# mmetcalf14/qml-cutensornet

Hardware: AMD Instinct MI355X
Metric: Gram kernel entries/sec @ 60 qubits x 6 layers (higher is better)
Workload: dtype f64 (complex128)

## Files before the change

### qml-cutensornet_amd/csrc/qk_fused.h

```cpp
#pragma once
#include "qk_device.h"

#define QKF_PRIO_LO() __builtin_amdgcn_s_setprio(0)
#define QKF_PRIO_HI() __builtin_amdgcn_s_setprio(2)
typedef double v2d __attribute__((ext_vector_type(2)));
typedef __attribute__((address_space(3))) v2d lds_v2d;
static constexpr int QKF_XSTEP = 4 * TILE;
static constexpr int QKF_XBLOCK = TILE * TILE;


#ifndef QKF_LDS3M
#define QKF_LDS3M 0
#endif
#ifndef QKF_P2_PROBE
#define QKF_P2_PROBE 0
#endif
#ifndef QKF_ABL
#define QKF_ABL 0
#endif
#define QKF_STEP_BARRIER()                            \
  do {                                                \
    if (QKF_ABL & 4) asm volatile("s_waitcnt lgkmcnt(0)" ::: "memory"); \
    else qk_lds_barrier();                            \
  } while (0)
#define QKF_SUM(a, b) ((QKF_ABL & 1) ? (a) : (a) + (b))
#define QKF_DIF(a, b) ((QKF_ABL & 1) ? (b) : (a) - (b))
template <bool CONJB>
__device__ __forceinline__ void qkf_kstep(v4d& p1, v4d& p2, v4d& p3, const double ar, const double ai, const double br, const double bi) {
  const double sa = QKF_SUM(ar, ai), sb = CONJB ? QKF_DIF(br, bi) : QKF_SUM(br, bi);
  p1 = __builtin_amdgcn_mfma_f64_16x16x4f64(ar, br, p1, 0, 0, 0);
  p2 = __builtin_amdgcn_mfma_f64_16x16x4f64(ai, bi, p2, 0, 0, 0);
  p3 = __builtin_amdgcn_mfma_f64_16x16x4f64(sa, sb, p3, 0, 0, 0);
}

struct QkfTile {
  v4d re, im;
};

__device__ __forceinline__ v2d qkf_ldg(const v2d* __restrict__ base, const unsigned off) {
  return *reinterpret_cast<const v2d*>(reinterpret_cast<const char*>(base) + (size_t)(off * 16u));
}
#ifndef QKF_NT_A
#define QKF_NT_A 0
#endif
#ifndef QKF_NT_B
#define QKF_NT_B 0
#endif
__device__ __forceinline__ v2d qkf_ldg_nt(const v2d* __restrict__ base, const unsigned off) {
  return __builtin_nontemporal_load(reinterpret_cast<const v2d*>(reinterpret_cast<const char*>(base) + (size_t)(off * 16u)));
}
__device__ __forceinline__ v2d qkf_ldg_a(const v2d* __restrict__ base, const unsigned off) { return QKF_NT_A ? qkf_ldg_nt(base, off) : qkf_ldg(base, off); }
__device__ __forceinline__ v2d qkf_ldg_b(const v2d* __restrict__ base, const unsigned off) { return QKF_NT_B ? qkf_ldg_nt(base, off) : qkf_ldg(base, off); }
__device__ __forceinline__ v2d qkf_ldx(const v2d* __restrict__ base, const unsigned off) { return qkf_ldg(base, off); }
__device__ __forceinline__ v2d qkf_ldx(const lds_v2d* base, const unsigned off) { return base[off]; }

struct QkfStream {
  const v2d* base;
  unsigned off;
  int step;
};
__device__ __forceinline__ void qkf_load4(v2d (&fr)[4], const QkfStream& st) {
#pragma unroll
  for (int i = 0; i < 4; ++i) fr[i] = qkf_ldg(st.base + i * st.step, st.off);
}

template <typename XPtr>
__device__ __forceinline__ void qkf_p1_tile(QkfTile& t, v2d (&fr)[4], const bool primed, QkfStream cur, XPtr xp, unsigned xoff, const int nks, const QkfStream nxt) {
  v4d p1 = {0, 0, 0, 0}, p2 = {0, 0, 0, 0}, p3 = {0, 0, 0, 0};
  v2d fx[4];
  if (!primed) qkf_load4(fr, cur);
#pragma unroll
  for (int i = 0; i < 4; ++i) fx[i] = qkf_ldx(xp + i * QKF_XSTEP, xoff);
  const int ng = (nks + 3) >> 2, last = nks - 4 * (ng - 1);
  QKF_PRIO_LO();
  int gq = 0;
  if (ng >= 2) {
    gq = 1;
    cur.off += 4 * cur.step, xoff += 4 * QKF_XSTEP;
#pragma unroll
    for (int i = 0; i < 4; ++i) {
      if (i == 0) {
        const v4d z = {0, 0, 0, 0};
        p1 = __builtin_amdgcn_mfma_f64_16x16x4f64(fx[0].x, fr[0].x, z, 0, 0, 0);
        p2 = __builtin_amdgcn_mfma_f64_16x16x4f64(fx[0].y, fr[0].y, z, 0, 0, 0);
        p3 = __builtin_amdgcn_mfma_f64_16x16x4f64(QKF_SUM(fx[0].x, fx[0].y), QKF_SUM(fr[0].x, fr[0].y), z, 0, 0, 0);
      } else {
        qkf_kstep<false>(p1, p2, p3, fx[i].x, fx[i].y, fr[i].x, fr[i].y);
      }
      if (!(QKF_ABL & 2)) fr[i] = qkf_ldg_b(cur.base + i * cur.step, cur.off);
      if (!(QKF_ABL & 8)) fx[i] = qkf_ldx(xp + i * QKF_XSTEP, xoff);
      __builtin_amdgcn_sched_barrier(0);
    }
  }
#pragma unroll 1
  for (; gq + 1 < ng; ++gq) {
    cur.off += 4 * cur.step, xoff += 4 * QKF_XSTEP;
#pragma unroll
    for (int i = 0; i < 4; ++i) {
      qkf_kstep<false>(p1, p2, p3, fx[i].x, fx[i].y, fr[i].x, fr[i].y);
      if (!(QKF_ABL & 2)) fr[i] = qkf_ldg_b(cur.base + i * cur.step, cur.off);
      if (!(QKF_ABL & 8)) fx[i] = qkf_ldx(xp + i * QKF_XSTEP, xoff);
      __builtin_amdgcn_sched_barrier(0);
    }
  }
#pragma unroll
  for (int i = 0; i < 4; ++i) {
    if (i < last) qkf_kstep<false>(p1, p2, p3, fx[i].x, fx[i].y, fr[i].x, fr[i].y);
    if (!(QKF_ABL & 2)) fr[i] = qkf_ldg(nxt.base + i * nxt.step, nxt.off);
    __builtin_amdgcn_sched_barrier(0);
  }
  QKF_PRIO_HI();
  t.re = p1 - p2;
  t.im = p3 - p1 - p2;
}

typedef __attribute__((address_space(3))) int lds_int;
struct QkfTurn {
  lds_int* at;
  int idx;
  lds_int* broken;
  unsigned long long* gerr;
};
__device__ __forceinline__ void qkf_turn_add(__attribute__((address_space(3))) double* const d, const long rs, const v4d& re, const v4d& im, const QkfTurn& t, const int tn) {
  lds_int* const turn = t.at + tn;
  if (t.idx > 0) {
    int spins = 0;
#ifdef QKF_FIRST_STORE
    while (__builtin_amdgcn_readfirstlane(__hip_atomic_load(turn, __ATOMIC_RELAXED, __HIP_MEMORY_SCOPE_WORKGROUP)) == 0) {
#else
    while (__builtin_amdgcn_readfirstlane(__hip_atomic_load(turn, __ATOMIC_RELAXED, __HIP_MEMORY_SCOPE_WORKGROUP)) != t.idx) {
#endif
      __builtin_amdgcn_s_sleep(1);
      if (++spins > (1 << 20) || __builtin_amdgcn_readfirstlane(__hip_atomic_load(t.broken, __ATOMIC_RELAXED, __HIP_MEMORY_SCOPE_WORKGROUP)) != 0) {
        __hip_atomic_store(t.broken, 1, __ATOMIC_RELAXED, __HIP_MEMORY_SCOPE_WORKGROUP);
        if (t.gerr) *t.gerr = 1ull;
        break;
      }
    }
#pragma unroll
    for (int r = 0; r < 4; ++r) {
      __hip_atomic_fetch_add(d + r * rs, re[r], __ATOMIC_RELAXED, __HIP_MEMORY_SCOPE_WORKGROUP);
      __hip_atomic_fetch_add(d + r * rs + 1, im[r], __ATOMIC_RELAXED, __HIP_MEMORY_SCOPE_WORKGROUP);
    }
  } else {
#pragma unroll
    for (int r = 0; r < 4; ++r) *(lds_v2d*)(d + r * rs) = (v2d){re[r], im[r]};
  }
#ifdef QKF_FIRST_STORE
  if (t.idx > 0) return;
#endif
  asm volatile("s_waitcnt lgkmcnt(0)" ::: "memory");
  __hip_atomic_store(turn, t.idx + 1, __ATOMIC_RELAXED, __HIP_MEMORY_SCOPE_WORKGROUP);
}

template <bool FULL, bool DET = false>
__device__ __forceinline__ void qkf_p2_item(const QkfTile& t, v2d (&fr)[4], const bool primed, QkfStream cur, const int ps, const int nn, const int kmax, lds_v2d* xo, const int q,
                                            const int j, const QkfStream nxt, const QkfTurn turn = QkfTurn{nullptr, 0, nullptr, nullptr}) {
  if (!primed) qkf_load4(fr, cur);
  __attribute__((address_space(3))) double* d = (__attribute__((address_space(3))) double*)(xo + q * TILE + j);
#pragma unroll 1
  for (int tn = 0; tn < nn; ++tn) {
    v4d p1 = {0, 0, 0, 0}, p2 = {0, 0, 0, 0}, p3 = {0, 0, 0, 0};
    const bool fin = tn + 1 == nn;
    const v2d* const rb = fin ? nxt.base : cur.base;
    const int rs = fin ? nxt.step : cur.step;
    cur.off = fin ? nxt.off : cur.off + TILE;
    QKF_PRIO_LO();
#pragma unroll
    for (int i = 0; i < 4; ++i) {
      if (FULL || i < kmax) qkf_kstep<true>(p1, p2, p3, t.re[i], t.im[i], fr[i].x, fr[i].y);
      if (!(QKF_ABL & 2)) fr[i] = qkf_ldg_a(rb + i * rs, cur.off);
      __builtin_amdgcn_sched_barrier(0);
    }
    QKF_PRIO_HI();
    const v4d re = (QKF_ABL & 128) ? p1 : p1 + p2, im = (QKF_ABL & 128) ? p3 : p3 - p1 + p2;
    if constexpr (DET) qkf_turn_add(d, (long)2 * QKF_XSTEP, re, im, turn, tn);
    else if (QKF_ABL & 256) {
#pragma unroll
      for (int r = 0; r < 4; ++r) asm volatile("" ::"v"(re[r]), "v"(im[r]));
    } else {
#pragma unroll
      for (int r = 0; r < 4; ++r) {
        __hip_atomic_fetch_add(d + r * 2 * QKF_XSTEP, re[r], __ATOMIC_RELAXED, __HIP_MEMORY_SCOPE_WORKGROUP);
        __hip_atomic_fetch_add(d + r * 2 * QKF_XSTEP + 1, im[r], __ATOMIC_RELAXED, __HIP_MEMORY_SCOPE_WORKGROUP);
      }
    }
    d += 2 * ps;
  }
}

template <int S>
__device__ __forceinline__ void qkf_rotate(QkfTile (&T)[S], const int L) {
  if constexpr (S >= 2) {
    if (L == 2) {
      const QkfTile t = T[S - 2];
      T[S - 2] = T[S - 1], T[S - 1] = t;
    }
  }
  if constexpr (S >= 3) {
    if (L == 3) {
      const QkfTile t = T[S - 3];
      T[S - 3] = T[S - 2], T[S - 2] = T[S - 1], T[S - 1] = t;
    }
  }
  if constexpr (S >= 4) {
    if (L >= 4) {
      const QkfTile t0 = T[0];
#pragma unroll
      for (int e = 0; e + 1 < S; ++e) T[e] = T[e + 1];
      T[S - 1] = t0;
    }
  }
}

__device__ __forceinline__ void qkf_edge_tile(QkfTile& t, const v2d* __restrict__ Ay, const int ldy, const v2d* __restrict__ Ax, const int ldx, const int ks4) {
  v4d p1 = {0, 0, 0, 0}, p2 = {0, 0, 0, 0}, p3 = {0, 0, 0, 0};
  v2d fy[4], fx[4];
#pragma unroll
  for (int i = 0; i < 4; ++i) fy[i] = Ay[(long)(4 * i) * ldy], fx[i] = Ax[(long)(4 * i) * ldx];
  for (int s0 = 0; s0 < ks4; s0 += 4) {
    const bool more = s0 + 4 < ks4;
#pragma unroll
    for (int i = 0; i < 4; ++i) {
      qkf_kstep<true>(p1, p2, p3, fy[i].x, fy[i].y, fx[i].x, fx[i].y);
      if (more) fy[i] = Ay[(long)(4 * (s0 + 4 + i)) * ldy], fx[i] = Ax[(long)(4 * (s0 + 4 + i)) * ldx];
    }
  }
  t.re = p1 + p2, t.im = p3 - p1 + p2;
}

template <int NW, typename XOut>
__device__ __forceinline__ void qkf_edge_prefix(const SweepArgs& g, const int xi, const int yj, const int a, const int b, XOut xo, const int wave, const int q, const int j) {
  const v2d* const Lx = reinterpret_cast<const v2d*>(g.xedge) + g.xedge_offs[2 * (long long)xi];
  const v2d* const Ly = reinterpret_cast<const v2d*>(g.yedge) + g.yedge_offs[2 * (long long)yj];
  const int mt = a / TILE, nt = b / TILE, ks4 = (1 << g.edge_k) >> 2;
  for (int t = wave; t < mt * nt; t += NW) {
    const int tb = t / mt, ta = t - tb * mt;
    QkfTile T;
    qkf_edge_tile(T, Ly + (long)q * b + tb * TILE + j, b, Lx + (long)q * a + ta * TILE + j, a, ks4);
#pragma unroll
    for (int r = 0; r < 4; ++r) xo[ta * (b * TILE) + (tb * TILE + q + 4 * r) * TILE + j] = (v2d){T.re[r], T.im[r]};
  }
}

template <int NW, typename XIn>
__device__ __forceinline__ void qkf_edge_suffix(const SweepArgs& g, const int xi, const int yj, const int a, const int b, XIn xin, __attribute__((address_space(3))) double* zacc, const int wave,
                                                const int q, const int j) {
  const v2d* const Rx = reinterpret_cast<const v2d*>(g.xedge) + g.xedge_offs[2 * (long long)xi + 1];
  const v2d* const Ry = reinterpret_cast<const v2d*>(g.yedge) + g.yedge_offs[2 * (long long)yj + 1];
  const int mt = a / TILE, nt = b / TILE, ks4 = (1 << g.edge_k) >> 2;
  double zr = 0, zi = 0;
  for (int t = wave; t < mt * nt; t += NW) {
    const int tb = t / mt, ta = t - tb * mt;
    QkfTile T;
    qkf_edge_tile(T, Ry + (long)q * b + tb * TILE + j, b, Rx + (long)q * a + ta * TILE + j, a, ks4);
#pragma unroll
    for (int r = 0; r < 4; ++r) {
      const v2d x = xin[ta * (b * TILE) + (tb * TILE + q + 4 * r) * TILE + j];
      zr += x.x * T.re[r] - x.y * T.im[r], zi += x.x * T.im[r] + x.y * T.re[r];
    }
  }
#pragma unroll
  for (int o = 32; o > 0; o >>= 1) zr += __shfl_xor(zr, o), zi += __shfl_xor(zi, o);
  if ((q | j) == 0) zacc[2 * wave] = zr, zacc[2 * wave + 1] = zi;
}

struct QkfSite {
  int a, a2, b, b2, at, nks, mt, nt, nn, W, inv, pd, ps, next;
  bool small;
  const v2d *Ak, *Bk;
};
typedef int v4i __attribute__((ext_vector_type(4)));
typedef __attribute__((address_space(3))) v4i lds_v4i;

template <int XCAP, int NT, typename OneRound>
__device__ __forceinline__ void qkf_step_table(const SweepArgs& g, const int xi, const int yj, lds_v4i* const rec, long long* const m_off, const int tid, const OneRound one_round) {
  const int ns = g.n_sites, n1 = ns + 1;
  const int32_t* const xd = g.xdims + (long long)xi * n1;
  const int32_t* const yd = g.ydims + (long long)yj * n1;
  const int32_t* const xt = g.xtrue + (long long)xi * n1;
  const int32_t* const yt = g.ytrue + (long long)yj * n1;
  const v2d* const xdata = reinterpret_cast<const v2d*>(g.xdata);
  const v2d* const ydata = reinterpret_cast<const v2d*>(g.ydata);
  auto is_small = [&](const int a, const int a2, const int b, const int b2, const int pd) __attribute__((always_inline)) {
    return a * b <= XCAP && a2 * b2 <= XCAP && (one_round(pd * (a / TILE), b2 / TILE) || a * b + a2 * b2 <= XCAP);
  };
  auto put = [&](const int e, const int a, const int a2, const int b, const int b2, const int ps, const int next, const bool small, const v2d* const A, const v2d* const B)
                 __attribute__((always_inline)) {
    const int mt = a / TILE, nt = b2 / TILE;
    const int W = small ? nt : max(1, min(nt, XCAP / (TILE * a2)));
    rec[3 * e] = (v4i){a, a2, b, b2};
    rec[3 * e + 1] = (v4i){xt[e], (yt[e] + 3) >> 2, W, small ? 1 : 0};
    rec[3 * e + 2] = (v4i){((1 << 20) + mt - 1) / mt, ps, next, 0};
    m_off[2 * e] = (long long)(((const char*)A - (const char*)xdata) / 16);
    m_off[2 * e + 1] = (long long)(((const char*)B - (const char*)ydata) / 16);
  };
  auto plain = [&](const int e, const int next) __attribute__((always_inline)) {
    const int a = xd[e], a2 = xd[e + 1], b = yd[e], b2 = yd[e + 1];
    put(e, a, a2, b, b2, 1, next, is_small(a, a2, b, b2, 2), xdata + (g.xoffs[(long long)xi * ns + e] >> 1), ydata + (g.yoffs[(long long)yj * ns + e] >> 1));
  };
  if (g.merge_steps == 0) {
    for (int e = tid; e < ns; e += NT) plain(e, e + 1);
    return;
  }
  const int ek = g.edge_k, k_hi = ns - ek;
  for (int t = tid; 2 * t < k_hi - ek; t += NT) {
    const int e = ek + 2 * t;
    if (e + 1 >= k_hi) {
      plain(e, e + 1);
      continue;
    }
    const int a = xd[e], am = xd[e + 1], a2 = xd[e + 2], b = yd[e], bm = yd[e + 1], b2 = yd[e + 2];
    const bool sm = is_small(a, a2, b, b2, 4);
    const long long work_m = 4ll * a * b2 * (b + a2), work_p = 2ll * a * bm * (b + am) + 2ll * am * b2 * (bm + a2);
    const bool merged = (sm || (!is_small(a, am, b, bm, 2) && !is_small(am, a2, bm, b2, 2))) && work_m <= work_p;
    plain(e + 1, e + 2);
    if (merged)
      put(e, a, a2, b, b2, 2, e + 2, sm, reinterpret_cast<const v2d*>(g.xmg) + (g.xmg_offs[(long long)xi * g.merge_steps + t] >> 1),
          reinterpret_cast<const v2d*>(g.ymg) + (g.ymg_offs[(long long)yj * g.merge_steps + t] >> 1));
    else plain(e, e + 1);
  }
}

#ifdef QKF_PROF
#define QKF_PROF_DECL() \
  unsigned long long pf[8] = {0, 0, 0, 0, 0, 0, 0, 0}, pt = __builtin_amdgcn_s_memtime(); \
  const unsigned long long pt0 = pt
#define QKF_STAMP(i)                                              \
  do {                                                            \
    const unsigned long long now_ = __builtin_amdgcn_s_memtime(); \
    pf[i] += now_ - pt;                                           \
    pt = now_;                                                    \
  } while (0)
#define QKF_PROF_FLUSH()                                             \
  do {                                                               \
    if (lane == 0) {                                                 \
      pf[7] = __builtin_amdgcn_s_memtime() - pt0;                    \
      for (int i_ = 0; i_ < 8; ++i_) atomicAdd(g.prof + i_, pf[i_]); \
    }                                                                \
  } while (0)
#else
#define QKF_PROF_DECL()
#define QKF_STAMP(i)
#define QKF_PROF_FLUSH()
#endif

template <int NW, int S, int XCAP, int WPS, bool DET = false>
__global__ __launch_bounds__(64 * NW, WPS) void qk_sweep_fused_kernel(const SweepArgs g) {
  constexpr int NT = 64 * NW;
  extern __shared__ __attribute__((aligned(16))) double lds_raw[];
  lds_v2d* const XL = (lds_v2d*)lds_raw;
  long long* const slot = reinterpret_cast<long long*>(lds_raw + 2 * XCAP);
  const v2d* const xdata = reinterpret_cast<const v2d*>(g.xdata);
  const v2d* const ydata = reinterpret_cast<const v2d*>(g.ydata);
  v2d* const G0 = reinterpret_cast<v2d*>(g.scratch) + (long long)blockIdx.x * 2 * g.x_plane;
  const int tid = threadIdx.x, lane = tid & 63;
  const int wave = __builtin_amdgcn_readfirstlane(tid >> 6);
  const int j = lane & 15, q = lane >> 4;
  const int ns = g.n_sites;
  __attribute__((address_space(3))) double* const zacc = (__attribute__((address_space(3))) double*)(slot + 2);
  lds_v4i* const rec = (lds_v4i*)(slot + 2 + 32);
  long long* const m_off = reinterpret_cast<long long*>(slot + 2 + 32) + 6 * (long long)ns;
  lds_int* const tbroken = (lds_int*)(m_off + 2 * (long long)ns);
  lds_int* const turn0 = tbroken + 2;
  auto rfl = [&](const int v) __attribute__((always_inline)) { return __builtin_amdgcn_readfirstlane(v); };
  auto ldl = [&](const long long* p_) __attribute__((always_inline)) {
    const long long v = *p_;
    const unsigned lo = __builtin_amdgcn_readfirstlane((unsigned)v);
    const unsigned hi = __builtin_amdgcn_readfirstlane((unsigned)((unsigned long long)v >> 32));
    return (long long)(((unsigned long long)hi << 32) | lo);
  };
  auto site = [&](const int k) __attribute__((always_inline)) {
    const v4i r0 = rec[3 * k], r1 = rec[3 * k + 1], r2 = rec[3 * k + 2];
    QkfSite s;
    s.a = rfl(r0.x), s.a2 = rfl(r0.y), s.b = rfl(r0.z), s.b2 = rfl(r0.w);
    s.at = rfl(r1.x), s.nks = rfl(r1.y), s.W = rfl(r1.z), s.small = rfl(r1.w) != 0;
    s.inv = rfl(r2.x);
    s.ps = rfl(r2.y), s.pd = 1 << s.ps, s.next = rfl(r2.z);
    s.mt = s.a / TILE, s.nt = s.b2 / TILE, s.nn = s.a2 / TILE;
    s.Ak = xdata + ldl(m_off + 2 * k);
    s.Bk = ydata + ldl(m_off + 2 * k + 1);
    return s;
  };
  auto b_stream = [&](const QkfSite& s, const int s0, const int it) __attribute__((always_inline)) {
    const int pp = it & (s.pd - 1), u = it >> s.ps, tbl = (u * s.inv) >> 20;
    return QkfStream{s.Bk + pp * s.b2, (unsigned)((q * s.pd) * s.b2 + (s0 + tbl) * TILE + j), 4 * s.pd * s.b2};
  };
  auto a_stream = [&](const QkfSite& s, const int it) __attribute__((always_inline)) {
    const int pp = it & (s.pd - 1), u = it >> s.ps, tbl = (u * s.inv) >> 20, ta = u - tbl * s.mt;
    return QkfStream{s.Ak + pp * s.a2, (unsigned)(((ta * TILE + q) * s.pd) * s.a2 + j), 4 * s.pd * s.a2};
  };
  QKF_PROF_DECL();
  const int xcc = qk_xcc_id();
  int gang_round = 0;
  if (tid == 0) qk_tail_start(g);
  for (;;) {
    if (tid == 0) {
      const long long pp_ = qk_pull(g, xcc);
      qk_gang_sync(g, xcc, pp_ >= 0, gang_round);
      *slot = pp_;
    }
    __syncthreads();
    const long long p = *slot;
    __syncthreads();
    if (p < 0) break;
    const int xi = g.pairs[2 * p], yj = g.pairs[2 * p + 1];
    qkf_step_table<XCAP, NT>(g, xi, yj, rec, m_off, tid, [](const int pmt, const int nt) { return pmt * nt <= NW * S; });
    const int ek = g.edge_k, k_hi = ns - ek;
    const bool edges = ek > 0;
    if (!edges)
      for (int e = tid; e < TILE * TILE; e += NT) XL[e] = (v2d){e == 0 ? 1.0 : 0.0, 0.0};
    if constexpr (DET)
      for (int e = tid; e < 2 * g.turn_ints + 2; e += NT) tbroken[e] = 0;
    int tsel = 0;
    __syncthreads();
    bool xg = false;
    int cur = 0, xb = 0;
    if (edges) {
      const v4i r0 = rec[3 * ek];
      const int a_e = rfl(r0.x), b_e = rfl(r0.z);
      if (a_e * b_e <= XCAP) qkf_edge_prefix<NW>(g, xi, yj, a_e, b_e, XL, wave, q, j);
      else qkf_edge_prefix<NW>(g, xi, yj, a_e, b_e, G0, wave, q, j), xg = true;
      __syncthreads();
    }
    QKF_STAMP(0);
    QkfTile T[S];
    v2d fr[4];
    bool primed = false;
    QkfSite sn = site(ek);
    for (int k = ek; k < k_hi;) {
      const QkfSite sc = sn;
      k = sc.next;
      if (k < k_hi) sn = site(k);
      const int a = sc.a, a2 = sc.a2, b = sc.b, mt = sc.mt, nt = sc.nt, W = sc.W;
      const bool small = sc.small;
      v2d* const Gc = G0 + (long long)cur * g.x_plane;
      v2d* const Gn = G0 + (long long)(cur ^ 1) * g.x_plane;
      if (small && xg) {
        for (int e = tid; e < a * b; e += NT) XL[e] = Gc[e];
        __syncthreads();
        xg = false, xb = 0;
      } else if (!small && !xg) {
        for (int e = tid; e < a * b; e += NT) Gc[e] = XL[xb + e];
        __syncthreads();
        xg = true;
      }
      const int n_out = sc.b2 * a2;
      const bool pingpong = small && a * b + n_out <= XCAP;
      const int ob = !small ? 0 : pingpong ? (xb == 0 ? XCAP - n_out : 0) : 0;
      if (pingpong && !DET)
        for (int e = tid; e < n_out; e += NT) XL[ob + e] = (v2d){0.0, 0.0};
      QKF_STAMP(1);
      for (int s0 = 0; s0 < nt; s0 += W) {
        const int w = min(W, nt - s0), items = sc.pd * mt * w;
        lds_int* const tcur = turn0 + tsel * g.turn_ints;
        if constexpr (DET) {
          for (int e = tid; e < g.turn_ints; e += NT) turn0[(tsel ^ 1) * g.turn_ints + e] = 0;
        } else if (!small) {
          for (int e = tid; e < w * TILE * a2; e += NT) XL[e] = (v2d){0.0, 0.0};
          QKF_STEP_BARRIER();
        }
        QKF_STAMP(6);
        for (int r0 = 0; r0 < items; r0 += NW * S) {
          const int L = min(S, (items - r0 + NW - 1) / NW);
          const bool multi = L > 1;
          const int it0 = r0 + wave;
          auto phase1 = [&](auto xbase) __attribute__((always_inline)) {
#pragma unroll 1
            for (int s = 0; s < L; ++s) {
              if (multi) qkf_rotate<S>(T, L);
              const int it = it0 + NW * s;
              if (it < items) {
                const int u = it >> sc.ps, tbl = (u * sc.inv) >> 20, ta = u - tbl * mt;
                const bool more = s + 1 < L && it + NW < items;
                const QkfStream nxt = more ? b_stream(sc, s0, it + NW) : a_stream(sc, it0);
                qkf_p1_tile(T[S - 1], fr, primed, b_stream(sc, s0, it), xbase, (unsigned)(ta * (b * TILE) + q * TILE + j), sc.nks, nxt);
                primed = true;
              }
            }
          };
          if (xg) phase1((const v2d*)Gc);
          else phase1((const lds_v2d*)(XL + xb));
          QKF_STAMP(2);
          if (small && r0 == 0 && !(DET && pingpong)) {
            QKF_STEP_BARRIER();
            if (!pingpong && !DET) {
              for (int e = tid; e < n_out; e += NT) XL[e] = (v2d){0.0, 0.0};
              QKF_STEP_BARRIER();
            }
          }
          QKF_STAMP(3);
          const bool last_round = s0 + W >= nt && r0 + NW * S >= items;
#pragma unroll 1
          for (int s = 0; s < S; ++s) {
            const int it = it0 + NW * s;
            if (it >= items) break;
            if (multi) qkf_rotate<S>(T, L);
            const int u = it >> sc.ps, tbl = (u * sc.inv) >> 20, ta = u - tbl * mt;
            const int kmax = min(4, (sc.at - ta * TILE + 3) >> 2);
            const bool more = s + 1 < S && it + NW < items;
            const bool chain = !more && last_round && k < k_hi && wave < sn.pd * sn.mt * min(sn.W, sn.nt);
            const QkfStream nxt = more ? a_stream(sc, it + NW) : chain ? b_stream(sn, 0, wave) : a_stream(sc, it);
            const int tix = sc.pd * ta + (it & (sc.pd - 1));
            const QkfTurn turn{tcur + tbl * sc.nn, tix, tbroken, g.err};
            if (kmax == 4) qkf_p2_item<true, DET>(T[S - 1], fr, primed, a_stream(sc, it), w * QKF_XBLOCK, sc.nn, 4, XL + ob + tbl * QKF_XBLOCK, q, j, nxt, turn);
            else qkf_p2_item<false, DET>(T[S - 1], fr, primed, a_stream(sc, it), w * QKF_XBLOCK, sc.nn, kmax, XL + ob + tbl * QKF_XBLOCK, q, j, nxt, turn);
            primed = more || chain;
          }
          QKF_STAMP(4);
        }
        QKF_STEP_BARRIER();
        tsel ^= 1;
        QKF_STAMP(5);
        if (!small && nt > W) {
          for (int tn = 0; tn < sc.nn; ++tn)
            for (int e = tid; e < w * QKF_XBLOCK; e += NT) Gn[(long long)tn * (sc.b2 * TILE) + s0 * QKF_XBLOCK + e] = XL[tn * w * QKF_XBLOCK + e];
          __syncthreads();
          QKF_STAMP(1);
        }
      }
      if (!small) {
        if (nt > W) cur ^= 1;
        else xg = false, xb = 0;
      } else {
        xb = ob;
      }
    }
    if (edges) {
      const v4i r0 = rec[3 * (k_hi - 1)];
      const int a_e = rfl(r0.y), b_e = rfl(r0.w);
      if (xg) qkf_edge_suffix<NW>(g, xi, yj, a_e, b_e, (const v2d*)(G0 + (long long)cur * g.x_plane), zacc, wave, q, j);
      else qkf_edge_suffix<NW>(g, xi, yj, a_e, b_e, (const lds_v2d*)(XL + xb), zacc, wave, q, j);
      __syncthreads();
    }
    if (tid == 0) {
      v2d zz = {0.0, 0.0};
      if (edges)
        for (int w_ = 0; w_ < NW; ++w_) zz.x += zacc[2 * w_], zz.y += zacc[2 * w_ + 1];
      else zz = xg ? G0[(long long)cur * g.x_plane] : (v2d)XL[xb];
      g.values[p] = zz.x * zz.x + zz.y * zz.y;
      if (g.z) {
        g.z[2 * p] = zz.x;
        g.z[2 * p + 1] = zz.y;
      }
    }
    __syncthreads();
  }
  if (tid == 0) qk_tail_exit(g);
  QKF_PROF_FLUSH();
}

template <bool HAS1, typename XPtr>
__device__ __forceinline__ void qkf_p1_dual(QkfTile& t0, QkfTile& t1, v2d (&fr)[4], v2d (&fs)[4], const bool primed, QkfStream cur, XPtr xp, unsigned xoff, const int nks,
                                            const QkfStream nxt) {
  v4d p1 = {0, 0, 0, 0}, p2 = {0, 0, 0, 0}, p3 = {0, 0, 0, 0}, r1 = {0, 0, 0, 0}, r2 = {0, 0, 0, 0}, r3 = {0, 0, 0, 0};
  v2d fx[4];
  if (!primed) qkf_load4(fr, cur);
  if (HAS1) {
#pragma unroll
// ... 202 lines not shown
  }
  lds_double* d = (lds_double*)(xo + q * TILE + j);
  lds_double* d1 = d + 2 * QKF_XBLOCK;
  constexpr long rs = 2 * QKF_XSTEP;
  const v4d s0 = t0.re + t0.im, s1 = HAS1 ? t1.re + t1.im : s0;
  const v2d *const c0 = cur.base, *const c1 = cur.base + cur.step, *const c2 = cur.base + 2 * cur.step, *const c3 = cur.base + 3 * cur.step;
  unsigned off = cur.off;
#pragma unroll 1
  for (int tn = 0; tn + 1 < nn; ++tn) {
    off += TILE;
    qkf_p2_block<FULL, HAS1>(t0, t1, s0, s1, fr, kmax, c0, c1, c2, c3, off, d, d1, rs);
    d += 2 * ps, d1 += 2 * ps;
  }
  qkf_p2_block<FULL, HAS1>(t0, t1, s0, s1, fr, kmax, nxt.base, nxt.base + nxt.step, nxt.base + 2 * nxt.step, nxt.base + 3 * nxt.step, nxt.off, d, d1, rs);
}

template <int NW, int XCAP, int WPS, bool DET = false>
__global__ __launch_bounds__(64 * NW, WPS) void qk_sweep_fused_dual_kernel(const SweepArgs g) {
  constexpr int NT = 64 * NW;
  extern __shared__ __attribute__((aligned(16))) double lds_raw[];
  lds_v2d* const XL = (lds_v2d*)lds_raw;
  long long* const slot = reinterpret_cast<long long*>(lds_raw + 2 * XCAP);
  const v2d* const xdata = reinterpret_cast<const v2d*>(g.xdata);
  const v2d* const ydata = reinterpret_cast<const v2d*>(g.ydata);
  v2d* const G0 = reinterpret_cast<v2d*>(g.scratch) + (long long)blockIdx.x * 2 * g.x_plane;
  const int tid = threadIdx.x, lane = tid & 63;
  const int wave = __builtin_amdgcn_readfirstlane(tid >> 6);
  const int j = lane & 15, q = lane >> 4;
  const int ns = g.n_sites;
  __attribute__((address_space(3))) double* const zacc = (__attribute__((address_space(3))) double*)(slot + 2);
  lds_v4i* const rec = (lds_v4i*)(slot + 2 + 32);
  long long* const m_off = reinterpret_cast<long long*>(slot + 2 + 32) + 6 * (long long)ns;
  lds_int* const tbroken = (lds_int*)(m_off + 2 * (long long)ns);
  lds_int* const turn0 = tbroken + 2;
  auto rfl = [&](const int v) __attribute__((always_inline)) { return __builtin_amdgcn_readfirstlane(v); };
  auto ldl = [&](const long long* p_) __attribute__((always_inline)) {
    const long long v = *p_;
    const unsigned lo = __builtin_amdgcn_readfirstlane((unsigned)v);
    const unsigned hi = __builtin_amdgcn_readfirstlane((unsigned)((unsigned long long)v >> 32));
    return (long long)(((unsigned long long)hi << 32) | lo);
  };
  auto site = [&](const int k) __attribute__((always_inline)) {
    const v4i r0 = rec[3 * k], r1 = rec[3 * k + 1], r2 = rec[3 * k + 2];
    QkfSite s;
    s.a = rfl(r0.x), s.a2 = rfl(r0.y), s.b = rfl(r0.z), s.b2 = rfl(r0.w);
    s.at = rfl(r1.x), s.nks = rfl(r1.y), s.W = rfl(r1.z), s.small = rfl(r1.w) != 0;
    s.inv = rfl(r2.x);
    s.ps = rfl(r2.y), s.pd = 1 << s.ps, s.next = rfl(r2.z);
    s.mt = s.a / TILE, s.nt = s.b2 / TILE, s.nn = s.a2 / TILE;
    s.Ak = xdata + ldl(m_off + 2 * k);
    s.Bk = ydata + ldl(m_off + 2 * k + 1);
    return s;
  };
  auto b_stream = [&](const QkfSite& s, const int s0, const int v, const int half) __attribute__((always_inline)) {
    const int pp = v & (s.pd - 1), u = v >> s.ps, tp = (u * s.inv) >> 20;
    return QkfStream{s.Bk + pp * s.b2, (unsigned)((q * s.pd) * s.b2 + (s0 + 2 * tp + half) * TILE + j), 4 * s.pd * s.b2};
  };
  struct Unit {
    bool mine, has1;
    int v, half;
  };
  auto unit_of = [&](const QkfSite& s, const int w, const int units, const int r0) __attribute__((always_inline)) {
    Unit un;
    const int left = units - r0;
    const bool halves = 2 * left <= NW;
    un.half = (halves && wave >= left) ? 1 : 0;
    un.v = r0 + wave - (un.half ? left : 0);
    const int tp = ((un.v >> s.ps) * s.inv) >> 20;
    const bool second = 2 * tp + 1 < w;
    un.mine = un.v < units && (un.half == 0 || second);
    un.has1 = !halves && second;
    return un;
  };
  auto a_stream = [&](const QkfSite& s, const int v) __attribute__((always_inline)) {
    const int pp = v & (s.pd - 1), u = v >> s.ps, tp = (u * s.inv) >> 20, ta = u - tp * s.mt;
    return QkfStream{s.Ak + pp * s.a2, (unsigned)(((ta * TILE + q) * s.pd) * s.a2 + j), 4 * s.pd * s.a2};
  };
  QKF_PROF_DECL();
  const int xcc = qk_xcc_id();
  int gang_round = 0;
  if (tid == 0) qk_tail_start(g);
  for (;;) {
    if (tid == 0) {
      const long long pp_ = qk_pull(g, xcc);
      qk_gang_sync(g, xcc, pp_ >= 0, gang_round);
      *slot = pp_;
    }
    __syncthreads();
    const long long p = *slot;
    __syncthreads();
    if (p < 0) break;
    const int xi = g.pairs[2 * p], yj = g.pairs[2 * p + 1];
    qkf_step_table<XCAP, NT>(g, xi, yj, rec, m_off, tid, [](const int pmt, const int nt) { return pmt * ((nt + 1) / 2) <= NW; });
    const int ek = g.edge_k, k_hi = ns - ek;
    const bool edges = ek > 0;
    if (!edges)
      for (int e = tid; e < TILE * TILE; e += NT) XL[e] = (v2d){e == 0 ? 1.0 : 0.0, 0.0};
    if constexpr (DET)
      for (int e = tid; e < 2 * g.turn_ints + 2; e += NT) tbroken[e] = 0;
    int tsel = 0;
    __syncthreads();
    bool xg = false;
    int cur = 0, xb = 0;
    if (edges) {
      const v4i r0 = rec[3 * ek];
      const int a_e = rfl(r0.x), b_e = rfl(r0.z);
      if (a_e * b_e <= XCAP) qkf_edge_prefix<NW>(g, xi, yj, a_e, b_e, XL, wave, q, j);
      else qkf_edge_prefix<NW>(g, xi, yj, a_e, b_e, G0, wave, q, j), xg = true;
      __syncthreads();
    }
    QKF_STAMP(0);
    QkfTile T0, T1;
    v2d fr[4], fs[4];
    bool primed = false;
    QkfSite sn = site(ek);
    for (int k = ek; k < k_hi;) {
      const QkfSite sc = sn;
      k = sc.next;
      if (k < k_hi) sn = site(k);
      const int a = sc.a, a2 = sc.a2, b = sc.b, mt = sc.mt, nt = sc.nt, W = sc.W;
      const bool small = sc.small;
      v2d* const Gc = G0 + (long long)cur * g.x_plane;
      v2d* const Gn = G0 + (long long)(cur ^ 1) * g.x_plane;
      if (small && xg) {
        for (int e = tid; e < a * b; e += NT) XL[e] = Gc[e];
        __syncthreads();
        xg = false, xb = 0;
      } else if (!small && !xg) {
        for (int e = tid; e < a * b; e += NT) Gc[e] = XL[xb + e];
        __syncthreads();
        xg = true;
      }
      const int n_out = sc.b2 * a2;
      const bool pingpong = small && a * b + n_out <= XCAP;
      const int ob = !small ? 0 : pingpong ? (xb == 0 ? XCAP - n_out : 0) : 0;
      if (pingpong && !DET)
        for (int e = tid; e < n_out; e += NT) XL[ob + e] = (v2d){0.0, 0.0};
      QKF_STAMP(1);
      for (int s0 = 0; s0 < nt; s0 += W) {
        const int w = min(W, nt - s0), units = sc.pd * mt * ((w + 1) >> 1);
        lds_int* const tcur = turn0 + tsel * g.turn_ints;
        if constexpr (DET) {
          for (int e = tid; e < g.turn_ints; e += NT) turn0[(tsel ^ 1) * g.turn_ints + e] = 0;
        } else if (!small) {
          for (int e = tid; e < w * TILE * a2; e += NT) XL[e] = (v2d){0.0, 0.0};
          QKF_STEP_BARRIER();
        }
        for (int r0 = 0; r0 < units; r0 += NW) {
          const Unit un = unit_of(sc, w, units, r0);
          const int v = un.v;
          const bool mine = un.mine, has1 = un.has1;
          const int u = v >> sc.ps, tp = (u * sc.inv) >> 20, ta = u - tp * mt;
          if (mine) {
            const QkfStream bs = b_stream(sc, s0, v, un.half), as = a_stream(sc, v);
            const unsigned xoff = (unsigned)(ta * (b * TILE) + q * TILE + j);
            if (xg) {
              if (has1) qkf_p1_dual<true>(T0, T1, fr, fs, primed, bs, (const v2d*)Gc, xoff, sc.nks, as);
              else qkf_p1_dual<false>(T0, T1, fr, fs, primed, bs, (const v2d*)Gc, xoff, sc.nks, as);
            } else {
              if (has1) qkf_p1_dual<true>(T0, T1, fr, fs, primed, bs, (const lds_v2d*)(XL + xb), xoff, sc.nks, as);
              else qkf_p1_dual<false>(T0, T1, fr, fs, primed, bs, (const lds_v2d*)(XL + xb), xoff, sc.nks, as);
            }
          }
          QKF_STAMP(2);
          if (small && r0 == 0 && !(DET && pingpong)) {
            QKF_STEP_BARRIER();
            if (!pingpong && !DET) {
              for (int e = tid; e < n_out; e += NT) XL[e] = (v2d){0.0, 0.0};
              QKF_STEP_BARRIER();
            }
          }
          QKF_STAMP(3);
          if (mine) {
            const int kmax = min(4, (sc.at - ta * TILE + 3) >> 2);
            QkfStream nxt = a_stream(sc, v);
            bool np1 = false;
            if (r0 + NW < units) {
              const Unit nu = unit_of(sc, w, units, r0 + NW);
              if (nu.mine) nxt = b_stream(sc, s0, nu.v, nu.half), np1 = true;
            } else if (s0 + W < nt) {
              const int w2 = min(W, nt - s0 - W);
              const Unit nu = unit_of(sc, w2, sc.pd * mt * ((w2 + 1) >> 1), 0);
              if (nu.mine) nxt = b_stream(sc, s0 + W, nu.v, nu.half), np1 = true;
            } else if (k < k_hi) {
              const int w2 = min(sn.W, sn.nt);
              const Unit nu = unit_of(sn, w2, sn.pd * sn.mt * ((w2 + 1) >> 1), 0);
              if (nu.mine) nxt = b_stream(sn, 0, nu.v, nu.half), np1 = true;
            }
            const unsigned nd1 = 0;
            lds_v2d* const xo = XL + ob + (2 * tp + un.half) * QKF_XBLOCK;
            const QkfTurn tp_turn{tcur + (2 * tp + un.half) * sc.nn, sc.pd * ta + (v & (sc.pd - 1)), tbroken, g.err};
            if (has1) {
              if (kmax == 4) qkf_p2_dual<true, true, DET>(T0, T1, fr, fs, a_stream(sc, v), w * QKF_XBLOCK, sc.nn, 4, xo, q, j, nxt, np1, nd1, tp_turn);
              else qkf_p2_dual<false, true, DET>(T0, T1, fr, fs, a_stream(sc, v), w * QKF_XBLOCK, sc.nn, kmax, xo, q, j, nxt, np1, nd1, tp_turn);
            } else {
              if (kmax == 4) qkf_p2_dual<true, false, DET>(T0, T1, fr, fs, a_stream(sc, v), w * QKF_XBLOCK, sc.nn, 4, xo, q, j, nxt, np1, nd1, tp_turn);
              else qkf_p2_dual<false, false, DET>(T0, T1, fr, fs, a_stream(sc, v), w * QKF_XBLOCK, sc.nn, kmax, xo, q, j, nxt, np1, nd1, tp_turn);
            }
            primed = np1;
          }
          QKF_STAMP(4);
        }
        QKF_STEP_BARRIER();
        tsel ^= 1;
        QKF_STAMP(5);
        if (!small && nt > W) {
          for (int tn = 0; tn < sc.nn; ++tn)
            for (int e = tid; e < w * QKF_XBLOCK; e += NT) Gn[(long long)tn * (sc.b2 * TILE) + s0 * QKF_XBLOCK + e] = XL[tn * w * QKF_XBLOCK + e];
          __syncthreads();
        }
      }
      if (!small) {
        if (nt > W) cur ^= 1;
        else xg = false, xb = 0;
      } else {
        xb = ob;
      }
    }
    if (edges) {
      const v4i r0 = rec[3 * (k_hi - 1)];
      const int a_e = rfl(r0.y), b_e = rfl(r0.w);
      if (xg) qkf_edge_suffix<NW>(g, xi, yj, a_e, b_e, (const v2d*)(G0 + (long long)cur * g.x_plane), zacc, wave, q, j);
      else qkf_edge_suffix<NW>(g, xi, yj, a_e, b_e, (const lds_v2d*)(XL + xb), zacc, wave, q, j);
      __syncthreads();
    }
    if (tid == 0) {
      v2d zz = {0.0, 0.0};
      if (edges)
        for (int w_ = 0; w_ < NW; ++w_) zz.x += zacc[2 * w_], zz.y += zacc[2 * w_ + 1];
      else zz = xg ? G0[(long long)cur * g.x_plane] : (v2d)XL[xb];
      g.values[p] = zz.x * zz.x + zz.y * zz.y;
      if (g.z) {
        g.z[2 * p] = zz.x;
        g.z[2 * p + 1] = zz.y;
      }
    }
    __syncthreads();
    QKF_STAMP(6);
  }
  if (tid == 0) qk_tail_exit(g);
  QKF_PROF_FLUSH();
}

template <typename T>
// ... 221 lines not shown
```

### qml-cutensornet_amd/csrc/qk_plan.h

```cpp
#pragma once
#include "../../include/qkgram.h"

#include <algorithm>
#include <cstdint>
#include <cstdio>
#include <vector>

int qk_fail(int code, const char* fmt, ...) __attribute__((format(printf, 2, 3)));

#ifndef QKF_XCAP_ONE_V
#define QKF_XCAP_ONE_V 8192
#endif
#ifndef QKF_XCAP_TWO_V
#define QKF_XCAP_TWO_V 4608
#endif
#ifndef QKF_TWO_WGS
#define QKF_TWO_WGS 2
#endif
static constexpr int QKF_XCAP_ONE = QKF_XCAP_ONE_V, QKF_XCAP_TWO = QKF_XCAP_TWO_V;
static constexpr int QK_TILE = 16;
static inline int qk_pad16(int x) { return (x + QK_TILE - 1) / QK_TILE * QK_TILE; }
static constexpr int GMAX = 4;

struct qk_ctx;

struct qk_plan {
  int n_sites = 0, nx = 0, ny = 0;
  bool symmetric = false;
  bool quad = false;
  int world = 1, rank = 0;
  int64_t total_pairs = 0, max_per_rank = 0;
  std::vector<int32_t> pairs;
  std::vector<int32_t> groups;
  int group = 1;
  qk_stats stats{};
  qk_stats second{};
  int64_t n_first = 0;
  int nq = 1;
  int64_t qstart[17] = {0};
  int edge_k = 0;
  bool second_wave2 = false;
  double fit_two = 1.0;
  double fit_narrow = 1.0;
  double tile_reuse_bytes = 0;
  double plan_ms = 0;
  int plan_threads = 1;
  qk_ctx* up_ctx = nullptr;
  int32_t* d_pairs = nullptr;
  int32_t* d_groups = nullptr;
};

struct QkSweepPolicy {
  int variant = 20;
  int wgs_per_cu = 2;
  bool wave_path = true;
  bool wave2_ring = true;
  bool wave2_path = true;
  bool small_path = true;
  int fused_path = 1;
  int fused_split = 1;
  int fused_wgs = 0;
  bool deterministic = false;
  bool merge_sites = true;
  bool fused_dual = true;
  bool gang = false;
};

struct QkSetShape {
  int max_pad = 0, precision = 64, n_sites = 0;
};

struct QkSweepRun {
  int kernel = QK_KERNEL_NONE;
  long long grid = 0;
  size_t lds = 0;
// ... 93 lines not shown
```

Before: 701,600.

## Reorder fused work-item decode and clamp k-slab row pointers

Changes the non-deterministic fused kernel's work-item decode so that the tile-column index varies fastest before the padding plane, using precomputed 15-bit reciprocals for full and last strips. Row-stream pointers are clamped to valid k-slabs so loads past the real K extent re-read an in-range row instead of touching padding. The phase-1 inner loop now uses byte-offset cursors and splits into two passes so the final group uses clamped bases. This aims to cut wasted memory traffic on padded k-steps and improve locality across waves, at the cost of more index arithmetic and some added complexity.

Result: faster. 710,400, median of 6 (+1.3%).

```diff
diff --git a/qml-cutensornet_amd/csrc/qk_fused.h b/qml-cutensornet_amd/csrc/qk_fused.h
--- a/qml-cutensornet_amd/csrc/qk_fused.h
+++ b/qml-cutensornet_amd/csrc/qk_fused.h
@@ -1,5 +1,6 @@
 #pragma once
 #include "qk_device.h"
+#include "qk_plan.h"
 
 #define QKF_PRIO_LO() __builtin_amdgcn_s_setprio(0)
 #define QKF_PRIO_HI() __builtin_amdgcn_s_setprio(2)
@@ -58,25 +59,50 @@
   const v2d* base;
   unsigned off;
   int step;
+  int lim = 4;
 };
+__device__ __forceinline__ const v2d* qkf_kbase(const v2d* const base, const int step, const int i, const int lim) { return base + max(min(i, lim - 1), 0) * step; }
 __device__ __forceinline__ void qkf_load4(v2d (&fr)[4], const QkfStream& st) {
 #pragma unroll
-  for (int i = 0; i < 4; ++i) fr[i] = qkf_ldg(st.base + i * st.step, st.off);
-}
+  for (int i = 0; i < 4; ++i) fr[i] = qkf_ldg(qkf_kbase(st.base, st.step, i, st.lim), st.off);
+}
+__device__ __forceinline__ v2d qkf_ldgb(const v2d* __restrict__ base, const unsigned boff) {
+  const v2d* const at = reinterpret_cast<const v2d*>(reinterpret_cast<const char*>(base) + (size_t)boff);
+  return QKF_NT_B ? __builtin_nontemporal_load(at) : *at;
+}
+struct QkfXLds {
+  const lds_v2d* p;
+  __device__ __forceinline__ void advance() { p += 4 * QKF_XSTEP; }
+  __device__ __forceinline__ v2d kstep(const int i) const { return p[i * QKF_XSTEP]; }
+};
+struct QkfXGlobal {
+  const v2d* base;
+  unsigned bo;
+  __device__ __forceinline__ void advance() { bo += 4 * QKF_XSTEP * 16u; }
+  __device__ __forceinline__ v2d kstep(const int i) const { return *reinterpret_cast<const v2d*>(reinterpret_cast<const char*>(base + i * QKF_XSTEP) + (size_t)bo); }
+};
+__device__ __forceinline__ QkfXLds qkf_xcursor(const lds_v2d* xp, const unsigned xoff) { return QkfXLds{xp + xoff}; }
+__device__ __forceinline__ QkfXGlobal qkf_xcursor(const v2d* xp, const unsigned xoff) { return QkfXGlobal{xp, xoff * 16u}; }
 
 template <typename XPtr>
 __device__ __forceinline__ void qkf_p1_tile(QkfTile& t, v2d (&fr)[4], const bool primed, QkfStream cur, XPtr xp, unsigned xoff, const int nks, const QkfStream nxt) {
   v4d p1 = {0, 0, 0, 0}, p2 = {0, 0, 0, 0}, p3 = {0, 0, 0, 0};
   v2d fx[4];
+  const int ng = (nks + 3) >> 2, last = nks - 4 * (ng - 1);
   if (!primed) qkf_load4(fr, cur);
 #pragma unroll
   for (int i = 0; i < 4; ++i) fx[i] = qkf_ldx(xp + i * QKF_XSTEP, xoff);
-  const int ng = (nks + 3) >> 2, last = nks - 4 * (ng - 1);
+  const v2d* cb[4];
+#pragma unroll
+  for (int i = 0; i < 4; ++i) cb[i] = qkf_kbase(cur.base, cur.step, i, ng == 2 ? last : 4);
+  unsigned bo = cur.off * 16u;
+  const unsigned bs = (unsigned)(4 * cur.step) * 16u;
+  auto xq = qkf_xcursor(xp, xoff);
   QKF_PRIO_LO();
   int gq = 0;
   if (ng >= 2) {
     gq = 1;
-    cur.off += 4 * cur.step, xoff += 4 * QKF_XSTEP;
+    bo += bs, xq.advance();
 #pragma unroll
     for (int i = 0; i < 4; ++i) {
       if (i == 0) {
@@ -87,26 +113,32 @@
       } else {
         qkf_kstep<false>(p1, p2, p3, fx[i].x, fx[i].y, fr[i].x, fr[i].y);
       }
-      if (!(QKF_ABL & 2)) fr[i] = qkf_ldg_b(cur.base + i * cur.step, cur.off);
-      if (!(QKF_ABL & 8)) fx[i] = qkf_ldx(xp + i * QKF_XSTEP, xoff);
+      if (!(QKF_ABL & 2)) fr[i] = qkf_ldgb(cb[i], bo);
+      if (!(QKF_ABL & 8)) fx[i] = xq.kstep(i);
       __builtin_amdgcn_sched_barrier(0);
     }
   }
 #pragma unroll 1
-  for (; gq + 1 < ng; ++gq) {
-    cur.off += 4 * cur.step, xoff += 4 * QKF_XSTEP;
-#pragma unroll
-    for (int i = 0; i < 4; ++i) {
-      qkf_kstep<false>(p1, p2, p3, fx[i].x, fx[i].y, fr[i].x, fr[i].y);
-      if (!(QKF_ABL & 2)) fr[i] = qkf_ldg_b(cur.base + i * cur.step, cur.off);
-      if (!(QKF_ABL & 8)) fx[i] = qkf_ldx(xp + i * QKF_XSTEP, xoff);
-      __builtin_amdgcn_sched_barrier(0);
-    }
+  for (int pass = 0; pass < 2; ++pass) {
+    const int end = ng - 2 + pass;
+#pragma unroll 1
+    for (; gq < end; ++gq) {
+      bo += bs, xq.advance();
+#pragma unroll
+      for (int i = 0; i < 4; ++i) {
+        qkf_kstep<false>(p1, p2, p3, fx[i].x, fx[i].y, fr[i].x, fr[i].y);
+        if (!(QKF_ABL & 2)) fr[i] = qkf_ldgb(cb[i], bo);
+        if (!(QKF_ABL & 8)) fx[i] = xq.kstep(i);
+        __builtin_amdgcn_sched_barrier(0);
+      }
+    }
+#pragma unroll
+    for (int i = 0; i < 4; ++i) cb[i] = qkf_kbase(cur.base, cur.step, i, last);
   }
 #pragma unroll
   for (int i = 0; i < 4; ++i) {
     if (i < last) qkf_kstep<false>(p1, p2, p3, fx[i].x, fx[i].y, fr[i].x, fr[i].y);
-    if (!(QKF_ABL & 2)) fr[i] = qkf_ldg(nxt.base + i * nxt.step, nxt.off);
+    if (!(QKF_ABL & 2)) fr[i] = qkf_ldg(qkf_kbase(nxt.base, nxt.step, i, nxt.lim), nxt.off);
     __builtin_amdgcn_sched_barrier(0);
   }
   QKF_PRIO_HI();
@@ -163,13 +195,13 @@
     v4d p1 = {0, 0, 0, 0}, p2 = {0, 0, 0, 0}, p3 = {0, 0, 0, 0};
     const bool fin = tn + 1 == nn;
     const v2d* const rb = fin ? nxt.base : cur.base;
-    const int rs = fin ? nxt.step : cur.step;
+    const int rs = fin ? nxt.step : cur.step, rl = fin ? nxt.lim : FULL ? 4 : kmax;
     cur.off = fin ? nxt.off : cur.off + TILE;
     QKF_PRIO_LO();
 #pragma unroll
     for (int i = 0; i < 4; ++i) {
       if (FULL || i < kmax) qkf_kstep<true>(p1, p2, p3, t.re[i], t.im[i], fr[i].x, fr[i].y);
-      if (!(QKF_ABL & 2)) fr[i] = qkf_ldg_a(rb + i * rs, cur.off);
+      if (!(QKF_ABL & 2)) fr[i] = qkf_ldg_a(qkf_kbase(rb, rs, i, rl), cur.off);
       __builtin_amdgcn_sched_barrier(0);
     }
     QKF_PRIO_HI();
@@ -266,14 +298,14 @@
 }
 
 struct QkfSite {
-  int a, a2, b, b2, at, nks, mt, nt, nn, W, inv, pd, ps, next;
+  int a, a2, b, b2, at, nks, mt, nt, nn, W, inv, inv2, pd, ps, next;
   bool small;
   const v2d *Ak, *Bk;
 };
 typedef int v4i __attribute__((ext_vector_type(4)));
 typedef __attribute__((address_space(3))) v4i lds_v4i;
 
-template <int XCAP, int NT, typename OneRound>
+template <int XCAP, int NT, bool ITEM_RECIPS = false, typename OneRound>
 __device__ __forceinline__ void qkf_step_table(const SweepArgs& g, const int xi, const int yj, lds_v4i* const rec, long long* const m_off, const int tid, const OneRound one_round) {
   const int ns = g.n_sites, n1 = ns + 1;
   const int32_t* const xd = g.xdims + (long long)xi * n1;
@@ -291,7 +323,7 @@
     const int W = small ? nt : max(1, min(nt, XCAP / (TILE * a2)));
     rec[3 * e] = (v4i){a, a2, b, b2};
     rec[3 * e + 1] = (v4i){xt[e], (yt[e] + 3) >> 2, W, small ? 1 : 0};
-    rec[3 * e + 2] = (v4i){((1 << 20) + mt - 1) / mt, ps, next, 0};
+    rec[3 * e + 2] = (v4i){qk_recip20(mt), ps, next, ITEM_RECIPS ? qk_unit_recips(nt, W, false) : 0};
     m_off[2 * e] = (long long)(((const char*)A - (const char*)xdata) / 16);
     m_off[2 * e + 1] = (long long)(((const char*)B - (const char*)ydata) / 16);
   };
@@ -375,20 +407,23 @@
     QkfSite s;
     s.a = rfl(r0.x), s.a2 = rfl(r0.y), s.b = rfl(r0.z), s.b2 = rfl(r0.w);
     s.at = rfl(r1.x), s.nks = rfl(r1.y), s.W = rfl(r1.z), s.small = rfl(r1.w) != 0;
-    s.inv = rfl(r2.x);
+    s.inv = rfl(r2.x), s.inv2 = rfl(r2.w);
     s.ps = rfl(r2.y), s.pd = 1 << s.ps, s.next = rfl(r2.z);
     s.mt = s.a / TILE, s.nt = s.b2 / TILE, s.nn = s.a2 / TILE;
     s.Ak = xdata + ldl(m_off + 2 * k);
     s.Bk = ydata + ldl(m_off + 2 * k + 1);
     return s;
   };
-  auto b_stream = [&](const QkfSite& s, const int s0, const int it) __attribute__((always_inline)) {
-    const int pp = it & (s.pd - 1), u = it >> s.ps, tbl = (u * s.inv) >> 20;
-    return QkfStream{s.Bk + pp * s.b2, (unsigned)((q * s.pd) * s.b2 + (s0 + tbl) * TILE + j), 4 * s.pd * s.b2};
-  };
-  auto a_stream = [&](const QkfSite& s, const int it) __attribute__((always_inline)) {
-    const int pp = it & (s.pd - 1), u = it >> s.ps, tbl = (u * s.inv) >> 20, ta = u - tbl * s.mt;
-    return QkfStream{s.Ak + pp * s.a2, (unsigned)(((ta * TILE + q) * s.pd) * s.a2 + j), 4 * s.pd * s.a2};
+  auto item_of = [&](const QkfSite& s, const int w, const int it) __attribute__((always_inline)) {
+    return DET ? qk_unit_decode_ordered(it, s.ps, s.mt, s.inv) : qk_unit_decode(it, s.mt, w, s.inv, qk_unit_recip_of(s.inv2, w == s.W));
+  };
+  auto b_stream = [&](const QkfSite& s, const int s0, const int w, const int it) __attribute__((always_inline)) {
+    const QkUnit un = item_of(s, w, it);
+    return QkfStream{s.Bk + un.p * s.b2, (unsigned)((q * s.pd) * s.b2 + (s0 + un.tc) * TILE + j), 4 * s.pd * s.b2, min(4, s.nks)};
+  };
+  auto a_stream = [&](const QkfSite& s, const int w, const int it) __attribute__((always_inline)) {
+    const QkUnit un = item_of(s, w, it);
+    return QkfStream{s.Ak + un.p * s.a2, (unsigned)(((un.ta * TILE + q) * s.pd) * s.a2 + j), 4 * s.pd * s.a2, min(4, (s.at - un.ta * TILE + 3) >> 2)};
   };
   QKF_PROF_DECL();
   const int xcc = qk_xcc_id();
@@ -405,7 +440,7 @@
     __syncthreads();
     if (p < 0) break;
     const int xi = g.pairs[2 * p], yj = g.pairs[2 * p + 1];
-    qkf_step_table<XCAP, NT>(g, xi, yj, rec, m_off, tid, [](const int pmt, const int nt) { return pmt * nt <= NW * S; });
+    qkf_step_table<XCAP, NT, true>(g, xi, yj, rec, m_off, tid, [](const int pmt, const int nt) { return pmt * nt <= NW * S; });
     const int ek = g.edge_k, k_hi = ns - ek;
     const bool edges = ek > 0;
     if (!edges)
@@ -471,10 +506,10 @@
               if (multi) qkf_rotate<S>(T, L);
               const int it = it0 + NW * s;
               if (it < items) {
-                const int u = it >> sc.ps, tbl = (u * sc.inv) >> 20, ta = u - tbl * mt;
+                const int ta = item_of(sc, w, it).ta;
                 const bool more = s + 1 < L && it + NW < items;
-                const QkfStream nxt = more ? b_stream(sc, s0, it + NW) : a_stream(sc, it0);
-                qkf_p1_tile(T[S - 1], fr, primed, b_stream(sc, s0, it), xbase, (unsigned)(ta * (b * TILE) + q * TILE + j), sc.nks, nxt);
+                const QkfStream nxt = more ? b_stream(sc, s0, w, it + NW) : a_stream(sc, w, it0);
+                qkf_p1_tile(T[S - 1], fr, primed, b_stream(sc, s0, w, it), xbase, (unsigned)(ta * (b * TILE) + q * TILE + j), sc.nks, nxt);
                 primed = true;
               }
             }
@@ -496,15 +531,17 @@
             const int it = it0 + NW * s;
             if (it >= items) break;
             if (multi) qkf_rotate<S>(T, L);
-            const int u = it >> sc.ps, tbl = (u * sc.inv) >> 20, ta = u - tbl * mt;
+            const QkUnit un = item_of(sc, w, it);
+            const int ta = un.ta, tbl = un.tc;
             const int kmax = min(4, (sc.at - ta * TILE + 3) >> 2);
             const bool more = s + 1 < S && it + NW < items;
-            const bool chain = !more && last_round && k < k_hi && wave < sn.pd * sn.mt * min(sn.W, sn.nt);
-            const QkfStream nxt = more ? a_stream(sc, it + NW) : chain ? b_stream(sn, 0, wave) : a_stream(sc, it);
-            const int tix = sc.pd * ta + (it & (sc.pd - 1));
+            const int wn = min(sn.W, sn.nt);
+            const bool chain = !more && last_round && k < k_hi && wave < sn.pd * sn.mt * wn;
+            const QkfStream nxt = more ? a_stream(sc, w, it + NW) : chain ? b_stream(sn, 0, wn, wave) : a_stream(sc, w, it);
+            const int tix = sc.pd * ta + un.p;
             const QkfTurn turn{tcur + tbl * sc.nn, tix, tbroken, g.err};
-            if (kmax == 4) qkf_p2_item<true, DET>(T[S - 1], fr, primed, a_stream(sc, it), w * QKF_XBLOCK, sc.nn, 4, XL + ob + tbl * QKF_XBLOCK, q, j, nxt, turn);
-            else qkf_p2_item<false, DET>(T[S - 1], fr, primed, a_stream(sc, it), w * QKF_XBLOCK, sc.nn, kmax, XL + ob + tbl * QKF_XBLOCK, q, j, nxt, turn);
+            if (kmax == 4) qkf_p2_item<true, DET>(T[S - 1], fr, primed, a_stream(sc, w, it), w * QKF_XBLOCK, sc.nn, 4, XL + ob + tbl * QKF_XBLOCK, q, j, nxt, turn);
+            else qkf_p2_item<false, DET>(T[S - 1], fr, primed, a_stream(sc, w, it), w * QKF_XBLOCK, sc.nn, kmax, XL + ob + tbl * QKF_XBLOCK, q, j, nxt, turn);
             primed = more || chain;
           }
           QKF_STAMP(4);
@@ -813,9 +850,10 @@
     s.Bk = ydata + ldl(m_off + 2 * k + 1);
     return s;
   };
+  auto pair_of = [&](const QkfSite& s, const int v) __attribute__((always_inline)) { return qk_unit_decode_ordered(v, s.ps, s.mt, s.inv); };
   auto b_stream = [&](const QkfSite& s, const int s0, const int v, const int half) __attribute__((always_inline)) {
-    const int pp = v & (s.pd - 1), u = v >> s.ps, tp = (u * s.inv) >> 20;
-    return QkfStream{s.Bk + pp * s.b2, (unsigned)((q * s.pd) * s.b2 + (s0 + 2 * tp + half) * TILE + j), 4 * s.pd * s.b2};
+    const QkUnit un = pair_of(s, v);
+    return QkfStream{s.Bk + un.p * s.b2, (unsigned)((q * s.pd) * s.b2 + (s0 + 2 * un.tc + half) * TILE + j), 4 * s.pd * s.b2};
   };
   struct Unit {
     bool mine, has1;
@@ -827,15 +865,15 @@
     const bool halves = 2 * left <= NW;
     un.half = (halves && wave >= left) ? 1 : 0;
     un.v = r0 + wave - (un.half ? left : 0);
-    const int tp = ((un.v >> s.ps) * s.inv) >> 20;
+    const int tp = pair_of(s, un.v).tc;
     const bool second = 2 * tp + 1 < w;
     un.mine = un.v < units && (un.half == 0 || second);
     un.has1 = !halves && second;
     return un;
   };
   auto a_stream = [&](const QkfSite& s, const int v) __attribute__((always_inline)) {
-    const int pp = v & (s.pd - 1), u = v >> s.ps, tp = (u * s.inv) >> 20, ta = u - tp * s.mt;
-    return QkfStream{s.Ak + pp * s.a2, (unsigned)(((ta * TILE + q) * s.pd) * s.a2 + j), 4 * s.pd * s.a2};
+    const QkUnit un = pair_of(s, v);
+    return QkfStream{s.Ak + un.p * s.a2, (unsigned)(((un.ta * TILE + q) * s.pd) * s.a2 + j), 4 * s.pd * s.a2};
   };
   QKF_PROF_DECL();
   const int xcc = qk_xcc_id();
@@ -911,7 +949,8 @@
           const Unit un = unit_of(sc, w, units, r0);
           const int v = un.v;
           const bool mine = un.mine, has1 = un.has1;
-          const int u = v >> sc.ps, tp = (u * sc.inv) >> 20, ta = u - tp * mt;
+          const QkUnit pr = pair_of(sc, v);
+          const int tp = pr.tc, ta = pr.ta;
           if (mine) {
             const QkfStream bs = b_stream(sc, s0, v, un.half), as = a_stream(sc, v);
             const unsigned xoff = (unsigned)(ta * (b * TILE) + q * TILE + j);
@@ -950,7 +989,7 @@
             }
             const unsigned nd1 = 0;
             lds_v2d* const xo = XL + ob + (2 * tp + un.half) * QKF_XBLOCK;
-            const QkfTurn tp_turn{tcur + (2 * tp + un.half) * sc.nn, sc.pd * ta + (v & (sc.pd - 1)), tbroken, g.err};
+            const QkfTurn tp_turn{tcur + (2 * tp + un.half) * sc.nn, sc.pd * ta + pr.p, tbroken, g.err};
             if (has1) {
               if (kmax == 4) qkf_p2_dual<true, true, DET>(T0, T1, fr, fs, a_stream(sc, v), w * QKF_XBLOCK, sc.nn, 4, xo, q, j, nxt, np1, nd1, tp_turn);
               else qkf_p2_dual<false, true, DET>(T0, T1, fr, fs, a_stream(sc, v), w * QKF_XBLOCK, sc.nn, kmax, xo, q, j, nxt, np1, nd1, tp_turn);
diff --git a/qml-cutensornet_amd/csrc/qk_plan.h b/qml-cutensornet_amd/csrc/qk_plan.h
--- a/qml-cutensornet_amd/csrc/qk_plan.h
+++ b/qml-cutensornet_amd/csrc/qk_plan.h
@@ -21,6 +21,31 @@
 static constexpr int QK_TILE = 16;
 static inline int qk_pad16(int x) { return (x + QK_TILE - 1) / QK_TILE * QK_TILE; }
 static constexpr int GMAX = 4;
+
+#if defined(__HIPCC__)
+#define QK_HD __host__ __device__
+#else
+#define QK_HD
+#endif
+struct QkUnit {
+  int ta, tc, p;
+};
+QK_HD static inline int qk_unit_cols(const int w, const bool dual) { return dual ? (w + 1) >> 1 : w; }
+QK_HD static inline int qk_recip20(const int d) { return ((1 << 20) + d - 1) / d; }
+QK_HD static inline int qk_recip15(const int d) { return ((1 << 15) + d - 1) / d; }
+QK_HD static inline int qk_unit_recips(const int nt, const int W, const bool dual) {
+  const int wl = nt - (nt - 1) / W * W;
+  return qk_recip15(qk_unit_cols(W, dual)) | (qk_recip15(qk_unit_cols(wl, dual)) << 16);
+}
+QK_HD static inline int qk_unit_recip_of(const int recips, const bool full_strip) { return full_strip ? (recips & 0xffff) : (int)((unsigned)recips >> 16); }
+QK_HD static inline QkUnit qk_unit_decode(const int v, const int mt, const int wc, const int inv_mt, const int inv_wc) {
+  const int c = (v * inv_mt) >> 20, p = (c * inv_wc) >> 15;
+  return QkUnit{v - c * mt, c - p * wc, p};
+}
+QK_HD static inline QkUnit qk_unit_decode_ordered(const int v, const int ps, const int mt, const int inv_mt) {
+  const int u = v >> ps, tc = (u * inv_mt) >> 20;
+  return QkUnit{u - tc * mt, tc, v & ((1 << ps) - 1)};
+}
 
 struct qk_ctx;
 
```
